# Jittor/JNeRF

Hardware: AMD Instinct MI355X
Metric: training iters/s (higher is better)
Workload: dtype f32; 1 GPU; Instant-NGP lego config (projects/ngp/configs/ngp_base.py hyper-parameters: aabb_scale 1, L=16, T=2^19, F=2, fp32 table + fp32 field network (fp32-accurate products from split fp16 operands on the fp16 matrix cores: 2e-7 of the largest magnitude vs fp64 in forward and gradients, profiles/r03_split_accuracy.md), const_dt=True, 2^18-sample batches), procedural scene 'bricks' 100x800x800 RGBA (lego-d; scene=bricks, samples_per_iter_per_gpu=262144, parallelism=single

## Files before the change

jnerf_amd/csrc/sampler.hip:

```cpp
#include "ngp_common.h"
#include <stdlib.h>
#pragma clang fp contract(off)

struct MarchParams {
	float a0, a1, near_distance, cone_angle;
	int const_dt, cascades;
	uint64_t rng_state, rng_inc;
	const int32_t *occ_bounds;
	int occ_cascades;
	int occ_coarse;
};

__device__ __forceinline__ float clampf(float v, float lo, float hi) { return v < lo ? lo : (hi < v ? hi : v); }
__device__ __forceinline__ float max_cone_stepsize(int cascades) { return min_cone_stepsize() * (1 << (cascades - 1)) * NGP_STEPS / NGP_GRIDSIZE; }
__device__ __forceinline__ float calc_dt(float t, const MarchParams &p) {
	if (p.const_dt) return min_cone_stepsize() * 0.5;
	return clampf(t * p.cone_angle, min_cone_stepsize(), max_cone_stepsize(p.cascades));
}
__device__ __forceinline__ int mip_from_pos(const float pos[3], int cascades) {
	int e;
	float m = fmaxf(fmaxf(fabsf(pos[0] - 0.5f), fabsf(pos[1] - 0.5f)), fabsf(pos[2] - 0.5f));
	frexpf(m, &e);
	return min(cascades - 1, max(0, e + 1));
}
__device__ __forceinline__ int mip_from_dt(float dt, const float pos[3], int cascades) {
	int mip = mip_from_pos(pos, cascades);
	dt *= 2 * NGP_GRIDSIZE;
	if (dt < 1.f) return mip;
	int e; frexpf(dt, &e);
	return min(cascades - 1, max(e, mip));
}
__device__ __forceinline__ bool occupied_at(const float pos[3], const uint8_t *__restrict__ bitfield, uint32_t mip) {
	const float mip_scale = scalbnf(1.0f, -(int)mip);
	uint32_t c[3];
#pragma unroll
	for (int d = 0; d < 3; ++d) {
		float q = pos[d] - 0.5f; q *= mip_scale; q += 0.5f;
		int i = (int)(q * NGP_GRIDSIZE);
		c[d] = (uint32_t)min(max(i, 0), (int)NGP_GRIDSIZE - 1);
	}
	const uint32_t idx = morton3D(c[0], c[1], c[2]);
	return bitfield[idx / 8 + (NGP_GRIDSIZE * NGP_GRIDSIZE * NGP_GRIDSIZE * mip) / 8] & (1 << (idx % 8));
}
__device__ __forceinline__ float next_voxel_target(float t, const float pos[3], const float dir[3], const float idir[3], uint32_t res) {
	float t3[3];
#pragma unroll
	for (int d = 0; d < 3; ++d) {
		float q = res * pos[d];
		t3[d] = (floorf(q + 0.5f + 0.5f * copysignf(1.0f, dir[d])) - q) * idir[d];
	}
	float tt = fminf(fminf(t3[0], t3[1]), t3[2]);
	return t + fmaxf(tt / res, 0.0f);
}
__device__ __forceinline__ float advance_to_next_voxel(float t, const float pos[3], const float dir[3], const float idir[3], uint32_t res, const MarchParams &p) {
	const float t_target = next_voxel_target(t, pos, dir, idir, res);
	do { t += calc_dt(t, p); } while (t < t_target);
	return t;
}
__device__ __forceinline__ bool contains(const MarchParams &p, const float q[3]) {
	return q[0] >= p.a0 && q[0] <= p.a1 && q[1] >= p.a0 && q[1] <= p.a1 && q[2] >= p.a0 && q[2] <= p.a1;
}
__device__ __forceinline__ float ray_start(const MarchParams &p, uint32_t i, const float o[3], const float d[3]) {
	const float big = 3.402823466e+38f;
	float tmin = (p.a0 - o[0]) / d[0], tmax = (p.a1 - o[0]) / d[0];
	if (tmin > tmax) { float c = tmin; tmin = tmax; tmax = c; }
	float tymin = (p.a0 - o[1]) / d[1], tymax = (p.a1 - o[1]) / d[1];
	if (tymin > tymax) { float c = tymin; tymin = tymax; tymax = c; }
	bool miss = (tmin > tymax || tymin > tmax);
	if (!miss) {
		if (tymin > tmin) tmin = tymin;
		if (tymax < tmax) tmax = tymax;
		float tzmin = (p.a0 - o[2]) / d[2], tzmax = (p.a1 - o[2]) / d[2];
		if (tzmin > tzmax) { float c = tzmin; tzmin = tzmax; tzmax = c; }
		miss = (tmin > tzmax || tzmin > tmax);
		if (!miss && tzmin > tmin) tmin = tzmin;
	}
	if (miss) tmin = big;
	tmin = fmaxf(tmin, p.near_distance);
	Pcg32 rng{p.rng_state, p.rng_inc};
	rng.advance((uint64_t)(uint32_t)(i * 8u));
	float startt = tmin;
	startt += calc_dt(startt, p) * rng.next_float();
	return startt;
}

__device__ __forceinline__ bool occ_range(const MarchParams &p, const float o[3], const float d[3], float t_start, float &t_stop) {
	const float inf = __builtin_inff();
	bool any = false; t_stop = -inf;
	for (int c = 0; c < p.occ_cascades; ++c) {
		const int32_t *b = p.occ_bounds + c * 6;
		if (b[3] < b[0]) continue;
		const float sc = scalbnf(1.0f, c), cell = sc / NGP_GRIDSIZE;
		float tmin = t_start, tmax = inf;
		bool hit = true;
#pragma unroll
		for (int k = 0; k < 3; ++k) {
			const float lo = b[k] <= 0 ? -inf : 0.5f + ((float)b[k] / NGP_GRIDSIZE - 0.5f) * sc - 1.001f * cell;
			const float hi = b[3 + k] >= (int)NGP_GRIDSIZE - 1 ? inf : 0.5f + ((float)(b[3 + k] + 1) / NGP_GRIDSIZE - 0.5f) * sc + 1.001f * cell;
			if (d[k] == 0.0f) { if (o[k] < lo || o[k] > hi) hit = false; continue; }
// ... 2 lines not shown
			tmin = fmaxf(tmin, t0); tmax = fminf(tmax, t1);
		}
		if (hit && tmin <= tmax) { any = true; t_stop = fmaxf(t_stop, tmax); }
	}
	if (any) t_stop = t_stop + fabsf(t_stop) * 1e-5f + 1e-4f;
	return any;
}

__device__ __forceinline__ bool occ_coarse_range(const MarchParams &p, const float o[3], const float d[3], float t_start, float &t_stop, uint32_t lane) {
	const uint8_t *dil = reinterpret_cast<const uint8_t *>(p.occ_bounds + NGP_OCC_COARSE_OFFSET_INTS);
	{
		const int32_t *b1 = p.occ_bounds + 6;
		if (p.cascades > 1 && b1[3] >= b1[0] && (b1[0] < 32 || b1[1] < 32 || b1[2] < 32 || b1[3] > 95 || b1[4] > 95 || b1[5] > 95)) return true;
	}
	const float dn = sqrtf(d[0] * d[0] + d[1] * d[1] + d[2] * d[2]);
	if (!(dn > 0.f) || !(t_stop < 3.0e38f)) return true;
	const float h = (1.0f / NGP_OCC_COARSE) / dn * 0.999f;
	const float span = t_stop - t_start;
	const uint32_t n = (uint32_t)fminf(ceilf(span / h) + 2.0f, 4096.0f);
	float last = -__builtin_inff();
	for (uint32_t base = 0; base < n; base += 64u) {
		const float t = t_start + (float)(base + lane) * h;
		bool in = false;
		if (base + lane < n) {
			int c[3];
#pragma unroll
			for (int k = 0; k < 3; ++k) { const int q = (int)floorf((o[k] + t * d[k]) * NGP_OCC_COARSE); c[k] = min(max(q, 0), NGP_OCC_COARSE - 1); }
			in = dil[(c[2] * NGP_OCC_COARSE + c[1]) * NGP_OCC_COARSE + c[0]] != 0;
		}
		const unsigned long long m = __ballot(in);
		if (m) last = t_start + (float)(base + 63u - (uint32_t)__builtin_clzll(m)) * h;
	}
	if (last == -__builtin_inff()) return false;
	t_stop = fminf(t_stop, last + 2.0f * h + fabsf(last) * 1e-5f);
	return true;
}

#define NGP_TCACHE NGP_STEPS

template <bool WRITE>
__device__ __forceinline__ uint32_t march(const MarchParams &p, const uint8_t *__restrict__ bitfield, const float o[3], const float d[3], float startt,
                                          uint32_t limit, float *__restrict__ out, float *__restrict__ tcache = nullptr, uint32_t tstride = 0, float t_stop = __builtin_inff()) {
	const float idir[3] = {1.0f / d[0], 1.0f / d[1], 1.0f / d[2]};
	float wdir[3];
	if (WRITE) { wdir[0] = (d[0] + 1.0f) * 0.5f; wdir[1] = (d[1] + 1.0f) * 0.5f; wdir[2] = (d[2] + 1.0f) * 0.5f; }
	const float dtmin = min_cone_stepsize();
	const float dtspan = dtmin * (1 << (p.cascades - 1)) - dtmin;
	uint32_t j = 0; float t = startt; float pos[3];
	for (;;) {
#pragma unroll
		for (int k = 0; k < 3; ++k) pos[k] = o[k] + t * d[k];
		if (!(contains(p, pos) && j < limit) || t > t_stop) break;
		const float dt = calc_dt(t, p);
		const uint32_t mip = (uint32_t)mip_from_dt(dt, pos, p.cascades);
		if (occupied_at(pos, bitfield, mip)) {
			if (WRITE) {
				float *c = out + (size_t)j * 7;
#pragma unroll
				for (int k = 0; k < 3; ++k) c[k] = (pos[k] - p.a0) / (p.a1 - p.a0);
				c[3] = (dt - dtmin) / dtspan;
				c[4] = wdir[0]; c[5] = wdir[1]; c[6] = wdir[2];
			} else if (tcache) tcache[j] = t;
			++j; t += dt;
		} else {
			t = advance_to_next_voxel(t, pos, d, idir, NGP_GRIDSIZE >> mip, p);
		}
	}
	return j;
}

__global__ __launch_bounds__(128) void k_march_count(uint32_t n_rays, MarchParams p, const float *__restrict__ rays_o, const float *__restrict__ rays_d,
                                                     const uint8_t *__restrict__ bitfield, uint32_t *__restrict__ steps, float *__restrict__ startts) {
	const uint32_t i = blockIdx.x * blockDim.x + threadIdx.x;
	if (i >= n_rays) return;
	const float o[3] = {rays_o[3 * i], rays_o[3 * i + 1], rays_o[3 * i + 2]}, d[3] = {rays_d[3 * i], rays_d[3 * i + 1], rays_d[3 * i + 2]};
	const float startt = ray_start(p, i, o, d);
	float t_stop = __builtin_inff();
	if (p.occ_bounds && !occ_range(p, o, d, startt, t_stop)) { steps[i] = 0; return; }
	steps[i] = march<false>(p, bitfield, o, d, startt, NGP_STEPS, nullptr, startts ? startts + (size_t)i * NGP_TCACHE : nullptr, 1, t_stop);
}

#define MC_WIN 64u

__device__ __forceinline__ uint32_t wave_incl_max(uint32_t v, uint32_t lane) {
#pragma unroll
	for (int off = 1; off < 64; off <<= 1) { const uint32_t y = __shfl_up(v, off); if (lane >= (uint32_t)off) v = max(v, y); }
	return v;
}
__device__ __forceinline__ unsigned long long bits_below(uint32_t n) { return n >= 64u ? ~0ull : ((1ull << n) - 1ull); }

template <uint32_t NW, bool CONST_DT>
__global__ __launch_bounds__(64) void k_march_wave(uint32_t n_rays, MarchParams p, const float *__restrict__ rays_o, const float *__restrict__ rays_d,
                                                   const uint8_t *__restrict__ bitfield, uint32_t *__restrict__ steps, float *__restrict__ tcache) {
	constexpr uint32_t NC = NW * MC_WIN;
	__shared__ float tch[NC + 1];
	__shared__ uint32_t mlut[NGP_GRIDSIZE];
	__shared__ uint16_t wnext[NC];
	__shared__ float wtarget[NC];
	__shared__ unsigned long long wmask[NW][4];
	__shared__ uint32_t wres[3];
	const uint32_t lane = threadIdx.x, i = blockIdx.x;
	if (i >= n_rays) return;
	mlut[lane] = expand_bits(lane); mlut[lane + 64u] = expand_bits(lane + 64u);
	float o[3], d[3], idir[3], hs[3];
#pragma unroll
	for (int k = 0; k < 3; ++k) { o[k] = rays_o[3 * (size_t)i + k]; d[k] = rays_d[3 * (size_t)i + k]; idir[k] = 1.0f / d[k]; hs[k] = 0.5f * copysignf(1.0f, d[k]); }
	float t_round = ray_start(p, i, o, d);
	{
		float pos[3];
#pragma unroll
		for (int k = 0; k < 3; ++k) pos[k] = o[k] + t_round * d[k];
		if (!contains(p, pos)) { if (lane == 0) steps[i] = 0; return; }
	}
	float t_stop = __builtin_inff();
	if (p.occ_bounds && !occ_range(p, o, d, t_round, t_stop)) { if (lane == 0) steps[i] = 0; return; }
	if (p.occ_bounds && p.occ_coarse && !occ_coarse_range(p, o, d, t_round, t_stop, lane)) { if (lane == 0) steps[i] = 0; return; }
	const float big_neg = -__builtin_inff();
	uint32_t j0 = 0;
	float pend = big_neg;
	for (;;) {
		if (t_round > t_stop) { if (lane == 0) steps[i] = j0; return; }
		__syncthreads();
		if (CONST_DT) {
			const float dtc = calc_dt(t_round, p);
			uint32_t k = 0; float t = t_round;
			while (k <= NC) {
				int e; (void)frexpf(t, &e);
				const float sc = ldexpf(1.0f, 24 - e), a0f = t * sc;
				uint32_t m = 0, a0 = 0, q = 0;
				if (e > -100 && e < 100 && a0f >= 8388608.0f && a0f < 16777216.0f) {
					const float delta = dtc * sc;
					if (delta < 16777216.0f) {
						const float fl = floorf(delta);
						a0 = (uint32_t)a0f; q = (uint32_t)rintf(delta);
						const int X = (int)(16777215u - a0) - (int)(uint32_t)ceilf(delta);
						if (delta - fl != 0.5f && X >= 0 && q > 0u) m = (uint32_t)X / q + 1u;
					}
				}
				if (m == 0u) { if (lane == 0) tch[k] = t; t += dtc; ++k; continue; }
				const uint32_t last = min(m, NC - k);
				const float U = ldexpf(1.0f, e - 24);
				for (uint32_t c = lane; c <= last; c += 64u) tch[k + c] = (float)(a0 + c * q) * U;
				t = (float)(a0 + last * q) * U; k += last;
				if (k == NC) break;
			}
		} else if (lane == 0) {
			const float lo = min_cone_stepsize(), hi = max_cone_stepsize(p.cascades);
			float t = t_round;
#pragma unroll 8
			for (uint32_t k = 0; k <= NC; ++k) { tch[k] = t; t += clampf(t * p.cone_angle, lo, hi); }
		}
		__syncthreads();
		float tl[NW];
#pragma unroll
		for (uint32_t w = 0; w < NW; ++w) tl[w] = tch[w * MC_WIN + lane];
		t_round = tch[NC];
		uint32_t s = 0;
		if (pend != big_neg) {
			s = NC;
#pragma unroll
			for (int w = (int)NW - 1; w >= 0; --w) { const unsigned long long m = __ballot(!(tl[w] < pend)); if (m) s = (uint32_t)w * MC_WIN + (uint32_t)__builtin_ctzll(m); }
			if (s == NC) continue;
		}
		unsigned long long INm[NW], OCCm[NW];
		uint32_t nxw[NW]; float tgt[NW];
#pragma unroll
		for (uint32_t w = 0; w < NW; ++w) {
			const uint32_t self = w * MC_WIN + lane;
			nxw[w] = 0; tgt[w] = 0.f; INm[w] = 0ull; OCCm[w] = 0ull;
			if ((w + 1u) * MC_WIN <= s) continue;
			float pos[3];
#pragma unroll
			for (int k = 0; k < 3; ++k) pos[k] = o[k] + tl[w] * d[k];
			const bool inside = contains(p, pos);
			bool occ = false;
			float target = 0.f;
			uint32_t nx = self + 1u;
			if (inside) {
				const float dt = calc_dt(tl[w], p);
				const uint32_t mip = (uint32_t)mip_from_dt(dt, pos, p.cascades);
				const float mip_scale = scalbnf(1.0f, -(int)mip);
				uint32_t c[3];
#pragma unroll
				for (int k = 0; k < 3; ++k) {
					float q = pos[k] - 0.5f; q *= mip_scale; q += 0.5f;
					const int ci = (int)(q * NGP_GRIDSIZE);
					c[k] = (uint32_t)min(max(ci, 0), (int)NGP_GRIDSIZE - 1);
				}
				const uint32_t idx = mlut[c[0]] | (mlut[c[1]] << 1) | (mlut[c[2]] << 2);
				occ = bitfield[idx / 8 + (NGP_GRIDSIZE * NGP_GRIDSIZE * NGP_GRIDSIZE * mip) / 8] & (1 << (idx % 8));
				if (!occ) {
					const uint32_t res = NGP_GRIDSIZE >> mip;
					const float resf = (float)res, inv_res = scalbnf(1.0f, (int)mip - 7);
					float t3[3];
#pragma unroll
					for (int k = 0; k < 3; ++k) { const float q = resf * pos[k]; t3[k] = (floorf(q + 0.5f + hs[k]) - q) * idir[k]; }
					const float tt = fminf(fminf(t3[0], t3[1]), t3[2]);
					target = tl[w] + fmaxf(tt * inv_res, 0.0f);
					const float est = (target - tl[w]) * __frcp_rn(dt);
					uint32_t g = self + 1u;
					if (est > 1.0f) g = est >= (float)NC ? NC : self + (uint32_t)est;
					if (g > NC) g = NC;
					while (g > self + 1u && !(tch[g - 1u] < target)) --g;
					while (g < NC && tch[g] < target) ++g;
					nx = g;
				}
			}
			INm[w] = __ballot(inside); OCCm[w] = __ballot(occ);
			nxw[w] = nx; tgt[w] = target;
		}
		unsigned long long G[NW];
		{
			uint32_t carry = 0;
#pragma unroll
			for (uint32_t w = 0; w < NW; ++w) {
				const uint32_t self = w * MC_WIN + lane;
				const uint32_t incl = wave_incl_max(self >= s ? nxw[w] : 0u, lane);
				const uint32_t up = __shfl_up(incl, 1);
				const uint32_t ex = max(carry, lane ? up : 0u);
				G[w] = __ballot(self >= s && (self == s || ex == self));
				carry = max(carry, (uint32_t)__builtin_amdgcn_readlane((int)incl, 63));
			}
		}
		uint32_t FO = NC;
#pragma unroll
		for (int w = (int)NW - 1; w >= 0; --w) { const unsigned long long out = G[w] & ~INm[w]; if (out) FO = (uint32_t)w * MC_WIN + (uint32_t)__builtin_ctzll(out); }
		unsigned long long E[NW];
		bool bad = false;
		{
			uint32_t nfirst = NC;
#pragma unroll
			for (int w = (int)NW - 1; w >= 0; --w) {
				const uint32_t self = (uint32_t)w * MC_WIN + lane;
				const unsigned long long V = G[w] & INm[w] & bits_below(FO > (uint32_t)w * MC_WIN ? FO - (uint32_t)w * MC_WIN : 0u);
				const unsigned long long rest = lane == 63u ? 0ull : G[w] >> (lane + 1u);
				const uint32_t ng = rest ? self + 1u + (uint32_t)__builtin_ctzll(rest) : nfirst;
				if (__ballot(((V >> lane) & 1ull) && ng != nxw[w])) bad = true;
				E[w] = V & OCCm[w];
				if (G[w]) nfirst = (uint32_t)w * MC_WIN + (uint32_t)__builtin_ctzll(G[w]);
			}
		}
		uint32_t emitted = 0, fin = 0;
		if (!bad) {
			uint32_t total = 0;
#pragma unroll
			for (uint32_t w = 0; w < NW; ++w) total += (uint32_t)__builtin_popcountll(E[w]);
			const uint32_t room = NGP_STEPS - j0;
			if (total >= room) {
				uint32_t cum = 0;
#pragma unroll
				for (uint32_t w = 0; w < NW; ++w) {
					const uint32_t c = (uint32_t)__builtin_popcountll(E[w]);
					if (cum + c > room) {
						const uint32_t pre = (uint32_t)__builtin_popcountll(E[w] & bits_below(lane));
						E[w] = __ballot(((E[w] >> lane) & 1ull) && cum + pre < room);
					}
					cum += c;
				}
				emitted = room; fin = 1; pend = big_neg;
			} else {
				emitted = total; fin = FO < NC ? 1u : 0u; pend = big_neg;
				if (!fin) {
#pragma unroll
					for (int w = (int)NW - 1; w >= 0; --w) {
						if (G[w]) {
							const uint32_t ll = 63u - (uint32_t)__builtin_clzll(G[w]);
							if (!((OCCm[w] >> ll) & 1ull)) pend = __shfl(tgt[w], (int)ll);
							break;
						}
					}
				}
			}
		} else {
#pragma unroll
			for (uint32_t w = 0; w < NW; ++w) {
				const uint32_t self = w * MC_WIN + lane;
				const bool inside = (INm[w] >> lane) & 1ull, occ = (OCCm[w] >> lane) & 1ull;
				const unsigned long long NX = __ballot(inside && nxw[w] == self + 1u && (occ || nxw[w] < NC));
				wnext[self] = (uint16_t)nxw[w]; wtarget[self] = tgt[w];
				if (lane == 0) { wmask[w][0] = INm[w]; wmask[w][1] = OCCm[w]; wmask[w][2] = NX; wmask[w][3] = 0ull; }
			}
			__syncthreads();
			if (lane == 0) {
				uint32_t cur = s, em = 0, fn = 0;
				float new_pend = big_neg;
				while (cur < NC) {
					const uint32_t w = cur / MC_WIN, c = cur % MC_WIN;
					const unsigned long long IN = wmask[w][0], OCC = wmask[w][1], NX = wmask[w][2];
					if (!((IN >> c) & 1ull) || j0 + em >= NGP_STEPS) { fn = 1; break; }
					if ((NX >> c) & 1ull) {
						const unsigned long long rest = ~(NX >> c);
						uint32_t run = rest ? (uint32_t)__builtin_ctzll(rest) : 64u;
						if (run > MC_WIN - c) run = MC_WIN - c;
						const unsigned long long runmask = bits_below(run) << c;
						unsigned long long emm = OCC & runmask;
						const uint32_t n_em = (uint32_t)__builtin_popcountll(emm), room = NGP_STEPS - (j0 + em);
						if (n_em > room) {
							unsigned long long keep = 0ull;
							for (uint32_t q = 0; q < room; ++q) { const unsigned long long low = emm & (0ull - emm); keep |= low; emm ^= low; }
							wmask[w][3] |= keep; em += room; fn = 1;
							break;
						}
						wmask[w][3] |= emm; em += n_em; cur += run;
					} else {
						const uint32_t nx = wnext[cur];
						if (nx >= NC) { new_pend = wtarget[cur]; break; }
						cur = nx;
					}
				}
				wres[0] = em; wres[1] = fn; wres[2] = __float_as_uint(new_pend);
			}
			__syncthreads();
#pragma unroll
			for (uint32_t w = 0; w < NW; ++w) E[w] = wmask[w][3];
			emitted = wres[0]; fin = wres[1]; pend = __uint_as_float(wres[2]);
		}
		{
			uint32_t cum = j0;
#pragma unroll
			for (uint32_t w = 0; w < NW; ++w) {
				if (tcache && ((E[w] >> lane) & 1ull)) tcache[(size_t)i * NGP_TCACHE + cum + (uint32_t)__builtin_popcountll(E[w] & bits_below(lane))] = tl[w];
				cum += (uint32_t)__builtin_popcountll(E[w]);
			}
		}
		j0 += emitted;
		if (fin) { if (lane == 0) steps[i] = j0; return; }
	}
}

__device__ __forceinline__ uint32_t block_exclusive_scan_1024(uint32_t v, uint32_t *sh , uint32_t &total) {
	const uint32_t lane = threadIdx.x & 63u, wave = threadIdx.x >> 6;
	uint32_t x = v;
#pragma unroll
	for (int off = 1; off < 64; off <<= 1) { uint32_t y = __shfl_up(x, off); if (lane >= (uint32_t)off) x += y; }
	if (lane == 63) sh[wave] = x;
	__syncthreads();
	if (threadIdx.x == 0) { uint32_t acc = 0; for (int w = 0; w < 16; ++w) { uint32_t tcur = sh[w]; sh[w] = acc; acc += tcur; } sh[16] = acc; }
	__syncthreads();
	const uint32_t res = sh[wave] + x - v;
	total = sh[16];
	__syncthreads();
	return res;
}
#define MS_TILE 2048u
__device__ __forceinline__ uint32_t tiles_before(const uint32_t *__restrict__ tot, uint32_t b, uint32_t *sh) {
	uint32_t total;
	(void)block_exclusive_scan_1024(threadIdx.x < b ? tot[threadIdx.x] : 0u, sh, total);
	return total;
}
__global__ __launch_bounds__(1024) void k_mscan_totals(uint32_t n_rays, const uint32_t *__restrict__ steps, uint32_t *__restrict__ tot1) {
// ... 281 lines not shown
	for (uint32_t c0 = 0; c0 < ns; c0 += CG) {
		const uint32_t m = min(CG, ns - c0);
		float rgb[3] = {0.f, 0.f, 0.f}, alpha = 0.f;
		if (lane < m) {
			const size_t s = (size_t)base + c0 + lane;
			float o[4]; load4<T>(net + s * 4, o);
			const float dt = unwarp_dt(coords[s * 7 + 3], cascades);
			const float density = __expf(o[3]);
			alpha = 1.f - __expf(-density * dt);
#pragma unroll
			for (int c = 0; c < 3; ++c) rgb[c] = logistic(o[c]);
		}
		const float P = group_scan_mul<CG>(1.f - alpha, lane);
		float Pex = __shfl_up(P, 1, (int)CG); if (lane == 0) Pex = 1.f;
		const float weight = alpha * (T_ * Pex);
#pragma unroll
		for (int c = 0; c < 3; ++c) ray[c] += weight * rgb[c];
		T_ *= bcast<CG>(P, CG - 1u);
	}
#pragma unroll
	for (int c = 0; c < 3; ++c) ray[c] = group_sum<CG>(ray[c]);
	if (!INFERENCE && ns == numsteps[2 * i]) {
#pragma unroll
		for (int c = 0; c < 3; ++c) ray[c] += T_ * bg[3 * i + c];
	}
	if (lane == 0) {
#pragma unroll
		for (int c = 0; c < 3; ++c) rgb_out[3 * i + c] = ray[c];
		if (INFERENCE) alpha_out[i] = 1 - T_;
		if (!INFERENCE && hub.target) {
#pragma unroll
			for (int c = 0; c < 3; ++c) huber3(hub.target, hub.delta, hub.loss, hub.grad, i, (uint32_t)c, ray[c]);
		}
	}
}

template <typename T, uint32_t CG >
__global__ __launch_bounds__(256) void k_composite_bwd(uint32_t n_rays, const T *__restrict__ net, const float *__restrict__ coords, const uint32_t *__restrict__ numsteps_c,
                                                       const float *__restrict__ loss_grad, const float *__restrict__ rgb_ray, const float *__restrict__ density_grid_mean,
                                                       int cascades, T *__restrict__ dout) {
	const uint32_t lane = threadIdx.x & (CG - 1u), i = blockIdx.x * (256u / CG) + threadIdx.x / CG;
	if (i >= n_rays) return;
	float loss_scale = 128; loss_scale /= n_rays;
	const uint32_t ns = numsteps_c[2 * i], base = numsteps_c[2 * i + 1];
	if (ns == 0) return;
	const float l1 = *density_grid_mean < 0.01f ? 1e-4f : 0.0f;
	const float G[3] = {loss_grad[3 * i], loss_grad[3 * i + 1], loss_grad[3 * i + 2]}, R[3] = {rgb_ray[3 * i], rgb_ray[3 * i + 1], rgb_ray[3 * i + 2]};
	float T_ = 1.f, ray2[3] = {0.f, 0.f, 0.f};
	for (uint32_t c0 = 0; c0 < ns; c0 += CG) {
		const uint32_t m = min(CG, ns - c0);
		const size_t s = (size_t)base + c0 + lane;
		float o[4] = {0.f, 0.f, 0.f, 0.f}, rgb[3] = {0.f, 0.f, 0.f}, alpha = 0.f, dt = 0.f;
		if (lane < m) {
			load4<T>(net + s * 4, o);
#pragma unroll
			for (int c = 0; c < 3; ++c) rgb[c] = logistic(o[c]);
			dt = unwarp_dt(coords[s * 7 + 3], cascades);
			const float density = __expf(o[3]);
			alpha = 1.f - __expf(-density * dt);
		}
		const float P = group_scan_mul<CG>(1.f - alpha, lane);
		float Pex = __shfl_up(P, 1, (int)CG); if (lane == 0) Pex = 1.f;
		const float my_w = alpha * (T_ * Pex), my_T = T_ * P;
		float my_r2[3];
#pragma unroll
		for (int c = 0; c < 3; ++c) { const float S = group_scan_add<CG>(my_w * rgb[c], lane); my_r2[c] = ray2[c] + S; ray2[c] += bcast<CG>(S, CG - 1u); }
		T_ *= bcast<CG>(P, CG - 1u);
		if (lane < m) {
			float dl[4], dv[3];
#pragma unroll
			for (int c = 0; c < 3; ++c) {
				const float suffix = R[c] - my_r2[c];
				dl[c] = loss_scale * ((my_w * G[c]) * (rgb[c] * (1 - rgb[c])) + fmaxf(0.0f, 0.0f * o[c]));
				dv[c] = G[c] * (my_T * rgb[c] - suffix);
			}
			const float dotv = dv[0] + (dv[1] + dv[2]);
			const float dd = __expf(clampf(o[3], -15.0f, 15.0f));
			dl[3] = loss_scale * (dd * (dt * dotv)) + (o[3] < 0 ? -l1 : 0.0f);
			store4<T>(dout + s * 4, dl);
		}
	}
}

template <typename T, uint32_t CG >
__global__ __launch_bounds__(256) void k_composite_train(uint32_t n_rays, const T *__restrict__ net, const float *__restrict__ coords, const uint32_t *__restrict__ numsteps,
                                                         const uint32_t *__restrict__ numsteps_c, const float *__restrict__ bg, int cascades, float *__restrict__ rgb_out,
                                                         HuberArgs hub, const float *__restrict__ density_grid_mean, T *__restrict__ dout) {
	const uint32_t lane = threadIdx.x & (CG - 1u), i = blockIdx.x * (256u / CG) + threadIdx.x / CG;
	if (i >= n_rays) return;
	const uint32_t ns = numsteps_c[2 * i], base = numsteps_c[2 * i + 1];
	if (ns == 0) {
		if (lane < 3) {
			const float v = bg[3 * i + lane];
			rgb_out[3 * i + lane] = v;
			huber3(hub.target, hub.delta, hub.loss, hub.grad, i, lane, v);
		}
		return;
	}
	float T_ = 1.f, ray[3] = {0.f, 0.f, 0.f};
	float on[4] = {0.f, 0.f, 0.f, 0.f}, wn = 0.f;
	auto fetch = [&](uint32_t c0) { if (c0 + lane < ns) { const size_t s = (size_t)base + c0 + lane; load4<T>(net + s * 4, on); wn = coords[s * 7 + 3]; } };
	fetch(0);
	for (uint32_t c0 = 0; c0 < ns; c0 += CG) {
		const uint32_t m = min(CG, ns - c0);
		float rgb[3] = {0.f, 0.f, 0.f}, alpha = 0.f;
		const float o[4] = {on[0], on[1], on[2], on[3]}, wdt = wn;
		if (c0 + CG < ns) fetch(c0 + CG);
		if (lane < m) {
			const float dt = unwarp_dt(wdt, cascades);
			const float density = __expf(o[3]);
			alpha = 1.f - __expf(-density * dt);
#pragma unroll
			for (int c = 0; c < 3; ++c) rgb[c] = logistic(o[c]);
		}
		const float P = group_scan_mul<CG>(1.f - alpha, lane);
		float Pex = __shfl_up(P, 1, (int)CG); if (lane == 0) Pex = 1.f;
		const float weight = alpha * (T_ * Pex);
#pragma unroll
		for (int c = 0; c < 3; ++c) ray[c] += weight * rgb[c];
		T_ *= bcast<CG>(P, CG - 1u);
	}
#pragma unroll
	for (int c = 0; c < 3; ++c) ray[c] = group_sum<CG>(ray[c]);
	if (ns == numsteps[2 * i]) {
#pragma unroll
		for (int c = 0; c < 3; ++c) ray[c] += T_ * bg[3 * i + c];
	}
	float G[3];
#pragma unroll
	for (int c = 0; c < 3; ++c) {
		const float d = ray[c] - hub.target[3 * i + c], rel = fabsf(d);
		G[c] = rel > hub.delta ? (d > 0 ? 1.0f : -1.0f) : d / hub.delta;
		if (lane == 0) {
			rgb_out[3 * i + c] = ray[c];
			if (hub.loss) hub.loss[3 * i + c] = rel > hub.delta ? rel - 0.5f * hub.delta : 0.5f / hub.delta * rel * rel;
			hub.grad[3 * i + c] = G[c];
		}
	}
	float loss_scale = 128; loss_scale /= n_rays;
	const float l1 = *density_grid_mean < 0.01f ? 1e-4f : 0.0f;
	T_ = 1.f;
	float ray2[3] = {0.f, 0.f, 0.f};
	if (ns > CG) fetch(0);
	for (uint32_t c0 = 0; c0 < ns; c0 += CG) {
		const uint32_t m = min(CG, ns - c0);
		const size_t s = (size_t)base + c0 + lane;
		float o[4] = {0.f, 0.f, 0.f, 0.f}, rgb[3] = {0.f, 0.f, 0.f}, alpha = 0.f, dt = 0.f;
		const float oc[4] = {on[0], on[1], on[2], on[3]}, wdt = wn;
		if (c0 + CG < ns) fetch(c0 + CG);
		if (lane < m) {
			o[0] = oc[0]; o[1] = oc[1]; o[2] = oc[2]; o[3] = oc[3];
#pragma unroll
			for (int c = 0; c < 3; ++c) rgb[c] = logistic(o[c]);
			dt = unwarp_dt(wdt, cascades);
			const float density = __expf(o[3]);
			alpha = 1.f - __expf(-density * dt);
		}
		const float P = group_scan_mul<CG>(1.f - alpha, lane);
		float Pex = __shfl_up(P, 1, (int)CG); if (lane == 0) Pex = 1.f;
		const float my_w = alpha * (T_ * Pex), my_T = T_ * P;
		float my_r2[3];
#pragma unroll
		for (int c = 0; c < 3; ++c) { const float S = group_scan_add<CG>(my_w * rgb[c], lane); my_r2[c] = ray2[c] + S; ray2[c] += bcast<CG>(S, CG - 1u); }
		T_ *= bcast<CG>(P, CG - 1u);
		if (lane < m) {
			float dl[4], dv[3];
#pragma unroll
			for (int c = 0; c < 3; ++c) {
				const float suffix = ray[c] - my_r2[c];
				dl[c] = loss_scale * ((my_w * G[c]) * (rgb[c] * (1 - rgb[c])) + fmaxf(0.0f, 0.0f * o[c]));
				dv[c] = G[c] * (my_T * rgb[c] - suffix);
			}
			const float dotv = dv[0] + (dv[1] + dv[2]);
			const float dd = __expf(clampf(o[3], -15.0f, 15.0f));
			dl[3] = loss_scale * (dd * (dt * dotv)) + (o[3] < 0 ? -l1 : 0.0f);
			store4<T>(dout + s * 4, dl);
		}
	}
}

static int composite_fwd_impl(void *stream, uint32_t n_rays, const void *net, int dtype, const float *coords, const uint32_t *numsteps,
                              const uint32_t *numsteps_c, const float *bg, int cascades, float *rgb_out, HuberArgs hub);
NGP_API int ngp_composite_fwd(void *stream, uint32_t n_rays, const void *net, int dtype, const float *coords, const uint32_t *numsteps,
                              const uint32_t *numsteps_c, const float *bg, int cascades, float *rgb_out) {
	return composite_fwd_impl(stream, n_rays, net, dtype, coords, numsteps, numsteps_c, bg, cascades, rgb_out, HuberArgs{nullptr, 0.f, nullptr, nullptr});
}
NGP_API int ngp_composite_fwd_huber(void *stream, uint32_t n_rays, const void *net, int dtype, const float *coords, const uint32_t *numsteps,
                                    const uint32_t *numsteps_c, const float *bg, int cascades, float *rgb_out, const float *target, float delta, float *loss, float *loss_grad) {
	NGP_REQUIRE(target && loss_grad, NGP_E_ARG, "ngp_composite_fwd_huber: null pointer");
	return composite_fwd_impl(stream, n_rays, net, dtype, coords, numsteps, numsteps_c, bg, cascades, rgb_out, HuberArgs{target, delta, loss, loss_grad});
}
static int composite_fwd_impl(void *stream, uint32_t n_rays, const void *net, int dtype, const float *coords, const uint32_t *numsteps,
                              const uint32_t *numsteps_c, const float *bg, int cascades, float *rgb_out, HuberArgs hub) {
	NGP_REQUIRE(net && coords && numsteps && numsteps_c && bg && rgb_out, NGP_E_ARG, "ngp_composite_fwd: null pointer");
	NGP_REQUIRE(dtype == NGP_F32 || dtype == NGP_F16, NGP_E_DTYPE, "ngp_composite_fwd: bad dtype %d", dtype);
	if (n_rays == 0) return 0;
	hipStream_t s = (hipStream_t)stream;
	const bool wide = (uint64_t)n_rays * 24u <= (1u << 18);
	const uint32_t cg = wide ? CG_INFER : CG_TRAIN;
	const dim3 grid(div_up(n_rays, 256u / cg)), block(256);
#define CF_GO(T, W) NGP_LAUNCH((k_composite_fwd<T, false, W>), grid, block, 0, s, n_rays, (const T *)net, coords, numsteps, numsteps_c, bg, cascades, rgb_out, (float *)nullptr, hub)
	if (dtype == NGP_F32) { if (wide) CF_GO(float, CG_INFER); else CF_GO(float, CG_TRAIN); }
	else { if (wide) CF_GO(__half, CG_INFER); else CF_GO(__half, CG_TRAIN); }
#undef CF_GO
	NGP_LAUNCH_CHECK("ngp_composite_fwd");
	return 0;
}
NGP_API int ngp_composite_inference(void *stream, uint32_t n_rays, const void *net, int dtype, const float *coords, const uint32_t *numsteps, int cascades,
                                    float *rgb_out, float *alpha_out) {
	NGP_REQUIRE(net && coords && numsteps && rgb_out && alpha_out, NGP_E_ARG, "ngp_composite_inference: null pointer");
	NGP_REQUIRE(dtype == NGP_F32 || dtype == NGP_F16, NGP_E_DTYPE, "ngp_composite_inference: bad dtype %d", dtype);
	if (n_rays == 0) return 0;
	const dim3 grid(div_up(n_rays, 256u / CG_INFER)), block(256);
	hipStream_t s = (hipStream_t)stream;
	if (dtype == NGP_F32) NGP_LAUNCH((k_composite_fwd<float, true, CG_INFER>), grid, block, 0, s, n_rays, (const float *)net, coords, numsteps, (const uint32_t *)nullptr, (const float *)nullptr, cascades, rgb_out, alpha_out, HuberArgs{nullptr, 0.f, nullptr, nullptr});
	else NGP_LAUNCH((k_composite_fwd<__half, true, CG_INFER>), grid, block, 0, s, n_rays, (const __half *)net, coords, numsteps, (const uint32_t *)nullptr, (const float *)nullptr, cascades, rgb_out, alpha_out, HuberArgs{nullptr, 0.f, nullptr, nullptr});
	NGP_LAUNCH_CHECK("ngp_composite_inference");
	return 0;
}
NGP_API int ngp_composite_bwd(void *stream, uint32_t n_rays, uint32_t n_elems, const void *net, int dtype, const float *coords, const uint32_t *numsteps_c,
                              const float *loss_grad, const float *rgb_ray, const float *density_grid_mean, int cascades, void *dout, int zero_first) {
	NGP_REQUIRE(net && coords && numsteps_c && loss_grad && rgb_ray && density_grid_mean && dout, NGP_E_ARG, "ngp_composite_bwd: null pointer");
	NGP_REQUIRE(dtype == NGP_F32 || dtype == NGP_F16, NGP_E_DTYPE, "ngp_composite_bwd: bad dtype %d", dtype);
	hipStream_t s = (hipStream_t)stream;
	if (zero_first) { hipError_t e = hipMemsetAsync(dout, 0, (size_t)n_elems * 4 * (dtype == NGP_F16 ? 2 : 4), s); if (e != hipSuccess) { ngp_set_error("ngp_composite_bwd memset: %s", hipGetErrorString(e)); return (int)e; } }
	if (n_rays == 0) return 0;
	const bool wide = (uint64_t)n_rays * 24u <= (uint64_t)n_elems;
	const uint32_t cg = wide ? CG_INFER : CG_TRAIN;
	const dim3 grid(div_up(n_rays, 256u / cg)), block(256);
#define CB_GO(T, W) NGP_LAUNCH((k_composite_bwd<T, W>), grid, block, 0, s, n_rays, (const T *)net, coords, numsteps_c, loss_grad, rgb_ray, density_grid_mean, cascades, (T *)dout)
	if (dtype == NGP_F32) { if (wide) CB_GO(float, CG_INFER); else CB_GO(float, CG_TRAIN); }
	else { if (wide) CB_GO(__half, CG_INFER); else CB_GO(__half, CG_TRAIN); }
#undef CB_GO
	NGP_LAUNCH_CHECK("ngp_composite_bwd");
	return 0;
}

NGP_API int ngp_composite_train(void *stream, uint32_t n_rays, uint32_t n_elems, const void *net, int dtype, const float *coords, const uint32_t *numsteps, const uint32_t *numsteps_c,
                                const float *bg, int cascades, float *rgb_out, const float *target, float delta, float *loss, float *loss_grad, const float *density_grid_mean, void *dout) {
	NGP_REQUIRE(net && coords && numsteps && numsteps_c && bg && rgb_out && target && loss_grad && density_grid_mean && dout, NGP_E_ARG, "ngp_composite_train: null pointer");
	NGP_REQUIRE(dtype == NGP_F32 || dtype == NGP_F16, NGP_E_DTYPE, "ngp_composite_train: bad dtype %d", dtype);
	if (n_rays == 0) return 0;
	hipStream_t s = (hipStream_t)stream;
	const bool wide = (uint64_t)n_rays * 24u <= (uint64_t)n_elems;
	const HuberArgs hub{target, delta, loss, loss_grad};
	if (wide != ((uint64_t)n_rays * 24u <= (1u << 18))) {
		const int e = composite_fwd_impl(stream, n_rays, net, dtype, coords, numsteps, numsteps_c, bg, cascades, rgb_out, hub);
		return e ? e : ngp_composite_bwd(stream, n_rays, n_elems, net, dtype, coords, numsteps_c, loss_grad, rgb_out, density_grid_mean, cascades, dout, 0);
	}
	const uint32_t cg = wide ? CG_INFER : CG_TRAIN;
	const dim3 grid(div_up(n_rays, 256u / cg)), block(256);
#define CT_GO(T, W) NGP_LAUNCH((k_composite_train<T, W>), grid, block, 0, s, n_rays, (const T *)net, coords, numsteps, numsteps_c, bg, cascades, rgb_out, hub, density_grid_mean, (T *)dout)
	if (dtype == NGP_F32) { if (wide) CT_GO(float, CG_INFER); else CT_GO(float, CG_TRAIN); }
	else { if (wide) CT_GO(__half, CG_INFER); else CT_GO(__half, CG_TRAIN); }
#undef CT_GO
	NGP_LAUNCH_CHECK("ngp_composite_train");
	return 0;
}

__global__ void k_huber(uint32_t n, const float *__restrict__ x, const float *__restrict__ target, float delta, float *__restrict__ loss, float *__restrict__ grad) {
	const uint32_t i = blockIdx.x * blockDim.x + threadIdx.x;
	if (i >= n) return;
	const float d = x[i] - target[i], rel = fabsf(d);
	if (loss) loss[i] = rel > delta ? rel - 0.5f * delta : 0.5f / delta * rel * rel;
	if (grad) grad[i] = rel > delta ? (d > 0 ? 1.0f : -1.0f) : d / delta;
}
NGP_API int ngp_huber(void *stream, uint32_t n, const float *x, const float *target, float delta, float *loss, float *grad) {
	NGP_REQUIRE(x && target && (loss || grad), NGP_E_ARG, "ngp_huber: null pointer");
	if (n == 0) return 0;
	NGP_LAUNCH(k_huber, dim3(div_up(n, 256)), dim3(256), 0, (hipStream_t)stream, n, x, target, delta, loss, grad);
	NGP_LAUNCH_CHECK("ngp_huber");
	return 0;
}
```

Measured before the change: 2271 iters/s.

## Add cooperative block compositing for long rays and hoist per-ray loads early

Splits the fused composite-train kernel into a per-wavefront path and an optional cooperative path where all wavefronts in a block share one long ray, passing segment transmittance and colour prefix sums through LDS. The cooperative path is enabled only through the NGP_COMPOSITE_COOP environment variable and defaults to off. The default path now also issues the numsteps, background, target and density-mean loads before the marching loop when CG is 64, so their latency can overlap it. The cost is more registers and some extra work on short rays.

```diff
diff --git a/jnerf_amd/csrc/sampler.hip b/jnerf_amd/csrc/sampler.hip
--- a/jnerf_amd/csrc/sampler.hip
+++ b/jnerf_amd/csrc/sampler.hip
@@ -814,13 +814,11 @@
 	}
 }
 
+
 template <typename T, uint32_t CG >
-__global__ __launch_bounds__(256) void k_composite_train(uint32_t n_rays, const T *__restrict__ net, const float *__restrict__ coords, const uint32_t *__restrict__ numsteps,
-                                                         const uint32_t *__restrict__ numsteps_c, const float *__restrict__ bg, int cascades, float *__restrict__ rgb_out,
-                                                         HuberArgs hub, const float *__restrict__ density_grid_mean, T *__restrict__ dout) {
-	const uint32_t lane = threadIdx.x & (CG - 1u), i = blockIdx.x * (256u / CG) + threadIdx.x / CG;
-	if (i >= n_rays) return;
-	const uint32_t ns = numsteps_c[2 * i], base = numsteps_c[2 * i + 1];
+__device__ __forceinline__ void composite_train_own(uint32_t i, uint32_t lane, uint32_t ns, uint32_t base, uint32_t n_rays, const T *__restrict__ net, const float *__restrict__ coords,
+                                                    const uint32_t *__restrict__ numsteps, const float *__restrict__ bg, int cascades, float *__restrict__ rgb_out,
+                                                    HuberArgs hub, const float *__restrict__ density_grid_mean, T *__restrict__ dout) {
 	if (ns == 0) {
 		if (lane < 3) {
 			const float v = bg[3 * i + lane];
@@ -833,6 +831,13 @@
 	float on[4] = {0.f, 0.f, 0.f, 0.f}, wn = 0.f;
 	auto fetch = [&](uint32_t c0) { if (c0 + lane < ns) { const size_t s = (size_t)base + c0 + lane; load4<T>(net + s * 4, on); wn = coords[s * 7 + 3]; } };
 	fetch(0);
+	constexpr bool EARLY = CG == 64;
+	uint32_t ns_all = 0; float bgv[3] = {0.f, 0.f, 0.f}, tg[3] = {0.f, 0.f, 0.f}, mean = 0.f;
+	if (EARLY) {
+		ns_all = numsteps[2 * i]; mean = *density_grid_mean;
+#pragma unroll
+		for (int c = 0; c < 3; ++c) { bgv[c] = bg[3 * i + c]; tg[c] = hub.target[3 * i + c]; }
+	}
 	for (uint32_t c0 = 0; c0 < ns; c0 += CG) {
 		const uint32_t m = min(CG, ns - c0);
 		float rgb[3] = {0.f, 0.f, 0.f}, alpha = 0.f;
@@ -854,14 +859,15 @@
 	}
 #pragma unroll
 	for (int c = 0; c < 3; ++c) ray[c] = group_sum<CG>(ray[c]);
-	if (ns == numsteps[2 * i]) {
-#pragma unroll
-		for (int c = 0; c < 3; ++c) ray[c] += T_ * bg[3 * i + c];
+	if (!EARLY) ns_all = numsteps[2 * i];
+	if (ns == ns_all) {
+#pragma unroll
+		for (int c = 0; c < 3; ++c) ray[c] += T_ * (EARLY ? bgv[c] : bg[3 * i + c]);
 	}
 	float G[3];
 #pragma unroll
 	for (int c = 0; c < 3; ++c) {
-		const float d = ray[c] - hub.target[3 * i + c], rel = fabsf(d);
+		const float d = ray[c] - (EARLY ? tg[c] : hub.target[3 * i + c]), rel = fabsf(d);
 		G[c] = rel > hub.delta ? (d > 0 ? 1.0f : -1.0f) : d / hub.delta;
 		if (lane == 0) {
 			rgb_out[3 * i + c] = ray[c];
@@ -870,7 +876,7 @@
 		}
 	}
 	float loss_scale = 128; loss_scale /= n_rays;
-	const float l1 = *density_grid_mean < 0.01f ? 1e-4f : 0.0f;
+	const float l1 = (EARLY ? mean : *density_grid_mean) < 0.01f ? 1e-4f : 0.0f;
 	T_ = 1.f;
 	float ray2[3] = {0.f, 0.f, 0.f};
 	if (ns > CG) fetch(0);
@@ -909,6 +915,211 @@
 			store4<T>(dout + s * 4, dl);
 		}
 	}
+}
+
+#ifndef NGP_COOP_KW
+#define NGP_COOP_KW 1
+#endif
+constexpr uint32_t COOP_BLOCK = 256;
+template <uint32_t RC> struct CoopLds { float P[RC], S[RC][3], wrgb[RC][3][64]; };
+template <typename T, uint32_t W , uint32_t COOP_ROUNDS >
+__device__ __forceinline__ void composite_train_long(CoopLds<COOP_ROUNDS> &L, uint32_t w, uint32_t lane, uint32_t i, uint32_t ns, uint32_t base, uint32_t n_rays, const T *__restrict__ net,
+                                                     const float *__restrict__ coords, const uint32_t *__restrict__ numsteps, const float *__restrict__ bg, int cascades,
+                                                     float *__restrict__ rgb_out, HuberArgs hub, const float *__restrict__ density_grid_mean, T *__restrict__ dout) {
+	constexpr uint32_t CG = 64, KW = COOP_ROUNDS / W;
+	static_assert(KW * W == COOP_ROUNDS && COOP_ROUNDS % 4 == 0, "the wavefront count divides the rounds of a block; LDS is read four rounds at a time");
+	const uint32_t n_rounds = (ns + CG - 1u) / CG;
+	float o[KW][4], wdt[KW];
+	auto fetch = [&](uint32_t rb, uint32_t nr) {
+#pragma unroll
+		for (uint32_t j = 0; j < KW; ++j) {
+			const uint32_t k = w + j * W, c0 = (rb + k) * CG;
+			o[j][0] = o[j][1] = o[j][2] = o[j][3] = 0.f; wdt[j] = 0.f;
+			if (k < nr && c0 + lane < ns) { const size_t s = (size_t)base + c0 + lane; load4<T>(net + s * 4, o[j]); wdt[j] = coords[s * 7 + 3]; }
+		}
+	};
+	fetch(0, min(COOP_ROUNDS, n_rounds));
+	const uint32_t ns_all = numsteps[2 * i];
+	const float mean = *density_grid_mean;
+	float bgv[3], tg[3];
+#pragma unroll
+	for (int c = 0; c < 3; ++c) { bgv[c] = bg[3 * i + c]; tg[c] = hub.target[3 * i + c]; }
+	float alpha[KW], rgb[KW][3], dt[KW], P[KW], Pex[KW], Tk[KW];
+	auto eval = [&](uint32_t rb, uint32_t nr) {
+#pragma unroll
+		for (uint32_t j = 0; j < KW; ++j) {
+			const uint32_t k = w + j * W, c0 = (rb + k) * CG;
+			alpha[j] = 0.f; dt[j] = 0.f; rgb[j][0] = rgb[j][1] = rgb[j][2] = 0.f; P[j] = Pex[j] = 1.f;
+			if (k < nr) {
+				if (c0 + lane < ns) {
+#pragma unroll
+					for (int c = 0; c < 3; ++c) rgb[j][c] = logistic(o[j][c]);
+					dt[j] = unwarp_dt(wdt[j], cascades);
+					const float density = __expf(o[j][3]);
+					alpha[j] = 1.f - __expf(-density * dt[j]);
+				}
+				P[j] = group_scan_mul<CG>(1.f - alpha[j], lane);
+				Pex[j] = __shfl_up(P[j], 1, (int)CG); if (lane == 0) Pex[j] = 1.f;
+				if (lane == CG - 1u) L.P[k] = P[j];
+			}
+		}
+	};
+	auto replay_T = [&](float &T_, uint32_t nr) {
+#pragma unroll
+		for (uint32_t j = 0; j < KW; ++j) Tk[j] = 0.f;
+		for (uint32_t k0 = 0; k0 < nr; k0 += 4) {
+#pragma unroll
+			for (uint32_t kk = k0; kk < k0 + 4; ++kk) {
+				const float p = L.P[kk];
+				if (kk < nr) {
+#pragma unroll
+					for (uint32_t j = 0; j < KW; ++j) if (kk == w + j * W) Tk[j] = T_;
+					T_ *= p;
+				}
+			}
+		}
+	};
+	float T_ = 1.f, ray[3] = {0.f, 0.f, 0.f};
+	for (uint32_t rb = 0; rb < n_rounds; rb += COOP_ROUNDS) {
+		const uint32_t nr = min(COOP_ROUNDS, n_rounds - rb);
+		if (rb) fetch(rb, nr);
+		eval(rb, nr);
+		__syncthreads();
+		replay_T(T_, nr);
+#pragma unroll
+		for (uint32_t j = 0; j < KW; ++j) {
+			const uint32_t k = w + j * W;
+			if (k < nr) {
+				const float weight = alpha[j] * (Tk[j] * Pex[j]);
+#pragma unroll
+				for (int c = 0; c < 3; ++c) L.wrgb[k][c][lane] = weight * rgb[j][c];
+			}
+		}
+		__syncthreads();
+		for (uint32_t k0 = 0; k0 < nr; k0 += 4) {
+#pragma unroll
+			for (uint32_t kk = k0; kk < k0 + 4; ++kk) {
+#pragma unroll
+				for (int c = 0; c < 3; ++c) { const float x = L.wrgb[kk][c][lane]; if (kk < nr) ray[c] += x; }
+			}
+		}
+	}
+#pragma unroll
+	for (int c = 0; c < 3; ++c) ray[c] = group_sum<CG>(ray[c]);
+	if (ns == ns_all) {
+#pragma unroll
+		for (int c = 0; c < 3; ++c) ray[c] += T_ * bgv[c];
+	}
+	float G[3];
+#pragma unroll
+	for (int c = 0; c < 3; ++c) {
+		const float d = ray[c] - tg[c], rel = fabsf(d);
+		G[c] = rel > hub.delta ? (d > 0 ? 1.0f : -1.0f) : d / hub.delta;
+		if (w == 0 && lane == 0) {
+			rgb_out[3 * i + c] = ray[c];
+			if (hub.loss) hub.loss[3 * i + c] = rel > hub.delta ? rel - 0.5f * hub.delta : 0.5f / hub.delta * rel * rel;
+			hub.grad[3 * i + c] = G[c];
+		}
+	}
+	float loss_scale = 128; loss_scale /= n_rays;
+	const float l1 = mean < 0.01f ? 1e-4f : 0.0f;
+	const bool one_block = n_rounds <= COOP_ROUNDS;
+	T_ = 1.f;
+	float ray2[3] = {0.f, 0.f, 0.f};
+	for (uint32_t rb = 0; rb < n_rounds; rb += COOP_ROUNDS) {
+		const uint32_t nr = min(COOP_ROUNDS, n_rounds - rb);
+		if (!one_block) {
+			fetch(rb, nr);
+			eval(rb, nr);
+			__syncthreads();
+			replay_T(T_, nr);
+		}
+		float my_w[KW], S[KW][3], r2k[KW][3];
+#pragma unroll
+		for (uint32_t j = 0; j < KW; ++j) {
+			const uint32_t k = w + j * W;
+			my_w[j] = 0.f;
+#pragma unroll
+			for (int c = 0; c < 3; ++c) S[j][c] = r2k[j][c] = 0.f;
+			if (k < nr) {
+				my_w[j] = alpha[j] * (Tk[j] * Pex[j]);
+#pragma unroll
+				for (int c = 0; c < 3; ++c) { S[j][c] = group_scan_add<CG>(my_w[j] * rgb[j][c], lane); if (lane == CG - 1u) L.S[k][c] = S[j][c]; }
+			}
+		}
+		__syncthreads();
+		for (uint32_t k0 = 0; k0 < nr; k0 += 4) {
+#pragma unroll
+			for (uint32_t kk = k0; kk < k0 + 4; ++kk) {
+#pragma unroll
+				for (int c = 0; c < 3; ++c) {
+					const float x = L.S[kk][c];
+					if (kk < nr) {
+#pragma unroll
+						for (uint32_t j = 0; j < KW; ++j) if (kk == w + j * W) r2k[j][c] = ray2[c];
+						ray2[c] += x;
+					}
+				}
+			}
+		}
+#pragma unroll
+		for (uint32_t j = 0; j < KW; ++j) {
+			const uint32_t k = w + j * W, c0 = (rb + k) * CG;
+			if (k < nr && c0 + lane < ns) {
+				const size_t s = (size_t)base + c0 + lane;
+				const float my_T = Tk[j] * P[j];
+				float dl[4], dv[3];
+#pragma unroll
+				for (int c = 0; c < 3; ++c) {
+					const float my_r2 = r2k[j][c] + S[j][c];
+					const float suffix = ray[c] - my_r2;
+					dl[c] = loss_scale * ((my_w[j] * G[c]) * (rgb[j][c] * (1 - rgb[j][c])) + fmaxf(0.0f, 0.0f * o[j][c]));
+					dv[c] = G[c] * (my_T * rgb[j][c] - suffix);
+				}
+				const float dotv = dv[0] + (dv[1] + dv[2]);
+				const float dd = __expf(clampf(o[j][3], -15.0f, 15.0f));
+				dl[3] = loss_scale * (dd * (dt[j] * dotv)) + (o[j][3] < 0 ? -l1 : 0.0f);
+				store4<T>(dout + s * 4, dl);
+			}
+		}
+	}
+}
+
+template <typename T, uint32_t CG , uint32_t COOP>
+__global__ __launch_bounds__(COOP ? COOP : 256) void k_composite_train(uint32_t n_rays, const T *__restrict__ net, const float *__restrict__ coords, const uint32_t *__restrict__ numsteps,
+                                                                       const uint32_t *__restrict__ numsteps_c, const float *__restrict__ bg, int cascades, float *__restrict__ rgb_out,
+                                                                       HuberArgs hub, const float *__restrict__ density_grid_mean, T *__restrict__ dout) {
+	constexpr uint32_t BS = COOP ? COOP : 256u;
+	const uint32_t lane = threadIdx.x & (CG - 1u), i = blockIdx.x * (BS / CG) + threadIdx.x / CG;
+#ifdef NGP_PROBE_COMPOSITE_CLAMP
+#define COMPOSITE_NS(x) min(x, CG)
+#else
+#define COMPOSITE_NS(x) (x)
+#endif
+	if constexpr (COOP == 0) {
+		if (i >= n_rays) return;
+		const uint32_t ns = COMPOSITE_NS(numsteps_c[2 * i]), base = numsteps_c[2 * i + 1];
+		composite_train_own<T, CG>(i, lane, ns, base, n_rays, net, coords, numsteps, bg, cascades, rgb_out, hub, density_grid_mean, dout);
+	} else {
+		static_assert(CG == 64, "a wavefront per ray");
+		constexpr uint32_t W = BS / 64u, RC = W * NGP_COOP_KW < 16u ? W * NGP_COOP_KW : 16u;
+		__shared__ CoopLds<RC> L;
+		__shared__ uint32_t noted[W][3];
+		const uint32_t w = __builtin_amdgcn_readfirstlane(threadIdx.x / 64u);
+		uint32_t ns = 0, base = 0;
+		if (i < n_rays) { ns = COMPOSITE_NS(numsteps_c[2 * i]); base = numsteps_c[2 * i + 1]; }
+		const bool is_long = ns > CG;
+		if (i < n_rays && !is_long) composite_train_own<T, CG>(i, lane, ns, base, n_rays, net, coords, numsteps, bg, cascades, rgb_out, hub, density_grid_mean, dout);
+		if (lane == 0) { noted[w][0] = is_long ? i : ~0u; noted[w][1] = ns; noted[w][2] = base; }
+		__syncthreads();
+		for (uint32_t v = 0; v < W; ++v) {
+			const uint32_t r = __builtin_amdgcn_readfirstlane(noted[v][0]);
+			if (r == ~0u) continue;
+			composite_train_long<T, W, RC>(L, w, lane, r, __builtin_amdgcn_readfirstlane(noted[v][1]), __builtin_amdgcn_readfirstlane(noted[v][2]), n_rays, net, coords, numsteps, bg,
+			                           cascades, rgb_out, hub, density_grid_mean, dout);
+		}
+	}
+#undef COMPOSITE_NS
 }
 
 static int composite_fwd_impl(void *stream, uint32_t n_rays, const void *net, int dtype, const float *coords, const uint32_t *numsteps,
@@ -980,11 +1191,14 @@
 		const int e = composite_fwd_impl(stream, n_rays, net, dtype, coords, numsteps, numsteps_c, bg, cascades, rgb_out, hub);
 		return e ? e : ngp_composite_bwd(stream, n_rays, n_elems, net, dtype, coords, numsteps_c, loss_grad, rgb_out, density_grid_mean, cascades, dout, 0);
 	}
-	const uint32_t cg = wide ? CG_INFER : CG_TRAIN;
-	const dim3 grid(div_up(n_rays, 256u / cg)), block(256);
-#define CT_GO(T, W) NGP_LAUNCH((k_composite_train<T, W>), grid, block, 0, s, n_rays, (const T *)net, coords, numsteps, numsteps_c, bg, cascades, rgb_out, hub, density_grid_mean, (T *)dout)
-	if (dtype == NGP_F32) { if (wide) CT_GO(float, CG_INFER); else CT_GO(float, CG_TRAIN); }
-	else { if (wide) CT_GO(__half, CG_INFER); else CT_GO(__half, CG_TRAIN); }
+	static const int coop_env = [] { const char *e = getenv("NGP_COMPOSITE_COOP"); return e ? atoi(e) : 0; }();
+	const uint32_t coop = !wide || coop_env == 0 ? 0u : coop_env == 1024 ? 1024u : coop_env == 256 ? 256u : COOP_BLOCK;
+	const uint32_t bs = coop ? coop : 256u;
+	const dim3 grid(div_up(n_rays, bs / (wide ? CG_INFER : CG_TRAIN))), block(bs);
+#define CT_GO(T, W, B) NGP_LAUNCH((k_composite_train<T, W, B>), grid, block, 0, s, n_rays, (const T *)net, coords, numsteps, numsteps_c, bg, cascades, rgb_out, hub, density_grid_mean, (T *)dout)
+#define CT_GO_T(T) do { if (!wide) CT_GO(T, CG_TRAIN, 0); else if (coop == 256u) CT_GO(T, CG_INFER, 256); else if (coop == 1024u) CT_GO(T, CG_INFER, 1024); else CT_GO(T, CG_INFER, 0); } while (0)
+	if (dtype == NGP_F32) CT_GO_T(float); else CT_GO_T(__half);
+#undef CT_GO_T
 #undef CT_GO
 	NGP_LAUNCH_CHECK("ngp_composite_train");
 	return 0;
```

Result: no change. 2270 iters/s, median of 2 (-0.0%).

## Batch occupancy bitfield loads and use DPP wave scans in march kernel

Applied to the files above, without the earlier changes.

Splits the per-window occupancy test into two passes: first compute all bitfield byte offsets for the NW sub-windows, then issue all bitfield loads together, then do the skip-target search. The aim is to overlap global memory latency across windows instead of serialising load then dependent compute. It also replaces the shfl_up-based inclusive max scan with DPP row-shift/broadcast ops, uses readlane instead of shfl for a uniform lane fetch, and makes calc_dt compile-time specialised on CONST_DT. These changes add register pressure from the extra per-window arrays and rely on AMDGPU-specific DPP control encodings.

```diff
diff --git a/jnerf_amd/csrc/sampler.hip b/jnerf_amd/csrc/sampler.hip
--- a/jnerf_amd/csrc/sampler.hip
+++ b/jnerf_amd/csrc/sampler.hip
@@ -15,6 +15,11 @@
 __device__ __forceinline__ float max_cone_stepsize(int cascades) { return min_cone_stepsize() * (1 << (cascades - 1)) * NGP_STEPS / NGP_GRIDSIZE; }
 __device__ __forceinline__ float calc_dt(float t, const MarchParams &p) {
 	if (p.const_dt) return min_cone_stepsize() * 0.5;
+	return clampf(t * p.cone_angle, min_cone_stepsize(), max_cone_stepsize(p.cascades));
+}
+template <bool CONST_DT>
+__device__ __forceinline__ float calc_dt_as(float t, const MarchParams &p) {
+	if (CONST_DT) return min_cone_stepsize() * 0.5;
 	return clampf(t * p.cone_angle, min_cone_stepsize(), max_cone_stepsize(p.cascades));
 }
 __device__ __forceinline__ int mip_from_pos(const float pos[3], int cascades) {
@@ -183,11 +188,18 @@
 
 #define MC_WIN 64u
 
-__device__ __forceinline__ uint32_t wave_incl_max(uint32_t v, uint32_t lane) {
-#pragma unroll
-	for (int off = 1; off < 64; off <<= 1) { const uint32_t y = __shfl_up(v, off); if (lane >= (uint32_t)off) v = max(v, y); }
+template <int CTRL, int ROW_MASK = 0xf>
+__device__ __forceinline__ uint32_t dpp_or_zero(uint32_t v) { return (uint32_t)__builtin_amdgcn_update_dpp(0, (int)v, CTRL, ROW_MASK, 0xf, false); }
+__device__ __forceinline__ uint32_t wave_incl_max(uint32_t v) {
+	v = max(v, dpp_or_zero<0x111>(v));
+	v = max(v, dpp_or_zero<0x112>(v));
+	v = max(v, dpp_or_zero<0x114>(v));
+	v = max(v, dpp_or_zero<0x118>(v));
+	v = max(v, dpp_or_zero<0x142, 0xa>(v));
+	v = max(v, dpp_or_zero<0x143, 0xc>(v));
 	return v;
 }
+__device__ __forceinline__ uint32_t wave_shr1_or_zero(uint32_t v) { return dpp_or_zero<0x138>(v); }
 __device__ __forceinline__ unsigned long long bits_below(uint32_t n) { return n >= 64u ? ~0ull : ((1ull << n) - 1ull); }
 
 template <uint32_t NW, bool CONST_DT>
@@ -223,7 +235,7 @@
 		if (t_round > t_stop) { if (lane == 0) steps[i] = j0; return; }
 		__syncthreads();
 		if (CONST_DT) {
-			const float dtc = calc_dt(t_round, p);
+			const float dtc = calc_dt_as<true>(t_round, p);
 			uint32_t k = 0; float t = t_round;
 			while (k <= NC) {
 				int e; (void)frexpf(t, &e);
@@ -263,22 +275,16 @@
 			for (int w = (int)NW - 1; w >= 0; --w) { const unsigned long long m = __ballot(!(tl[w] < pend)); if (m) s = (uint32_t)w * MC_WIN + (uint32_t)__builtin_ctzll(m); }
 			if (s == NC) continue;
 		}
-		unsigned long long INm[NW], OCCm[NW];
-		uint32_t nxw[NW]; float tgt[NW];
+		uint32_t occb[NW], meta[NW], boff[NW];
 #pragma unroll
 		for (uint32_t w = 0; w < NW; ++w) {
-			const uint32_t self = w * MC_WIN + lane;
-			nxw[w] = 0; tgt[w] = 0.f; INm[w] = 0ull; OCCm[w] = 0ull;
+			boff[w] = 0u; meta[w] = 0u;
 			if ((w + 1u) * MC_WIN <= s) continue;
 			float pos[3];
 #pragma unroll
 			for (int k = 0; k < 3; ++k) pos[k] = o[k] + tl[w] * d[k];
-			const bool inside = contains(p, pos);
-			bool occ = false;
-			float target = 0.f;
-			uint32_t nx = self + 1u;
-			if (inside) {
-				const float dt = calc_dt(tl[w], p);
+			if (contains(p, pos)) {
+				const float dt = calc_dt_as<CONST_DT>(tl[w], p);
 				const uint32_t mip = (uint32_t)mip_from_dt(dt, pos, p.cascades);
 				const float mip_scale = scalbnf(1.0f, -(int)mip);
 				uint32_t c[3];
@@ -289,23 +295,40 @@
 					c[k] = (uint32_t)min(max(ci, 0), (int)NGP_GRIDSIZE - 1);
 				}
 				const uint32_t idx = mlut[c[0]] | (mlut[c[1]] << 1) | (mlut[c[2]] << 2);
-				occ = bitfield[idx / 8 + (NGP_GRIDSIZE * NGP_GRIDSIZE * NGP_GRIDSIZE * mip) / 8] & (1 << (idx % 8));
-				if (!occ) {
-					const uint32_t res = NGP_GRIDSIZE >> mip;
-					const float resf = (float)res, inv_res = scalbnf(1.0f, (int)mip - 7);
-					float t3[3];
-#pragma unroll
-					for (int k = 0; k < 3; ++k) { const float q = resf * pos[k]; t3[k] = (floorf(q + 0.5f + hs[k]) - q) * idir[k]; }
-					const float tt = fminf(fminf(t3[0], t3[1]), t3[2]);
-					target = tl[w] + fmaxf(tt * inv_res, 0.0f);
-					const float est = (target - tl[w]) * __frcp_rn(dt);
-					uint32_t g = self + 1u;
-					if (est > 1.0f) g = est >= (float)NC ? NC : self + (uint32_t)est;
-					if (g > NC) g = NC;
-					while (g > self + 1u && !(tch[g - 1u] < target)) --g;
-					while (g < NC && tch[g] < target) ++g;
-					nx = g;
-				}
+				boff[w] = idx / 8 + (NGP_GRIDSIZE * NGP_GRIDSIZE * NGP_GRIDSIZE * mip) / 8;
+				meta[w] = 0x100u | (mip << 4) | (idx % 8);
+			}
+		}
+#pragma unroll
+		for (uint32_t w = 0; w < NW; ++w) occb[w] = bitfield[boff[w]];
+		unsigned long long INm[NW], OCCm[NW];
+		uint32_t nxw[NW]; float tgt[NW];
+#pragma unroll
+		for (uint32_t w = 0; w < NW; ++w) {
+			const uint32_t self = w * MC_WIN + lane;
+			nxw[w] = 0; tgt[w] = 0.f; INm[w] = 0ull; OCCm[w] = 0ull;
+			if ((w + 1u) * MC_WIN <= s) continue;
+			const bool inside = meta[w] != 0u;
+			const bool occ = inside && ((occb[w] >> (meta[w] & 7u)) & 1u);
+			float target = 0.f;
+			uint32_t nx = self + 1u;
+			if (inside && !occ) {
+				const uint32_t mip = (meta[w] >> 4) & 15u;
+				const float resf = (float)(NGP_GRIDSIZE >> mip), inv_res = scalbnf(1.0f, (int)mip - 7);
+				float t3[3];
+#pragma unroll
+				for (int k = 0; k < 3; ++k) { const float q = resf * (o[k] + tl[w] * d[k]); t3[k] = (floorf(q + 0.5f + hs[k]) - q) * idir[k]; }
+				const float tt = fminf(fminf(t3[0], t3[1]), t3[2]);
+				target = tl[w] + fmaxf(tt * inv_res, 0.0f);
+				const float dt = calc_dt_as<CONST_DT>(tl[w], p);
+				const float est = (target - tl[w]) * (CONST_DT ? 1.0f / dt : __builtin_amdgcn_rcpf(dt));
+				uint32_t g = self + 1u;
+				if (est > 1.0f) g = est >= (float)NC ? NC : self + (uint32_t)est;
+				if (g > NC) g = NC;
+				const float below = tch[g - 1u], at = tch[g];
+				if (g > self + 1u && !(below < target)) { do --g; while (g > self + 1u && !(tch[g - 1u] < target)); }
+				else if (g < NC && at < target) { do ++g; while (g < NC && tch[g] < target); }
+				nx = g;
 			}
 			INm[w] = __ballot(inside); OCCm[w] = __ballot(occ);
 			nxw[w] = nx; tgt[w] = target;
@@ -316,9 +339,8 @@
 #pragma unroll
 			for (uint32_t w = 0; w < NW; ++w) {
 				const uint32_t self = w * MC_WIN + lane;
-				const uint32_t incl = wave_incl_max(self >= s ? nxw[w] : 0u, lane);
-				const uint32_t up = __shfl_up(incl, 1);
-				const uint32_t ex = max(carry, lane ? up : 0u);
+				const uint32_t incl = wave_incl_max(self >= s ? nxw[w] : 0u);
+				const uint32_t ex = max(carry, wave_shr1_or_zero(incl));
 				G[w] = __ballot(self >= s && (self == s || ex == self));
 				carry = max(carry, (uint32_t)__builtin_amdgcn_readlane((int)incl, 63));
 			}
@@ -366,7 +388,7 @@
 					for (int w = (int)NW - 1; w >= 0; --w) {
 						if (G[w]) {
 							const uint32_t ll = 63u - (uint32_t)__builtin_clzll(G[w]);
-							if (!((OCCm[w] >> ll) & 1ull)) pend = __shfl(tgt[w], (int)ll);
+							if (!((OCCm[w] >> ll) & 1ull)) pend = __int_as_float(__builtin_amdgcn_readlane(__float_as_int(tgt[w]), (int)ll));
 							break;
 						}
 					}
```

New measurement: 2242 iters/s before, 2298 iters/s after (median of 6 runs). +2.5%, better.
